# ImIntheMiddle/EmLoco

Hardware: AMD Instinct MI355X
Metric: env-steps/sec (SMPL humanoid, num_envs) (higher is better)
Workload: dtype f32

## Files before the change

### emloco_amd/csrc/emloco_types.h

```cpp
#pragma once
#define EMLOCO_PART_WORDS 416
#include "../../include/emloco_sim.h"
#define EMLOCO_PART_TAG(seq, part) ((seq) * 4u + (unsigned)(part))
#define EMLOCO_ERR_PART_TIMEOUT 1u

#define EMLOCO_TOPO_PARENT 0
#define EMLOCO_TOPO_DEPTH 24
#define EMLOCO_TOPO_CHILD 48
#define EMLOCO_TOPO_PDPACK 120
#define EMLOCO_TOPO_CAND 144
#define EMLOCO_TOPO_SCPAIR 240
#define EMLOCO_TOPO_WORDS 560

#define EMLOCO_MB_DYN 0
#define EMLOCO_MB_GEO 384
#define EMLOCO_MB_CAP 576
#define EMLOCO_MB_DRV 832
#define EMLOCO_MODEL_WORDS 1112

struct EmlocoSimDev {
    int n_env, n_cand, max_depth, sc_n;
    int sc_nseg;
    const int *topo;
    const float *model;
// ... 23 lines not shown
```

### emloco_amd/csrc/sim_capi.hip

```cpp
#include <hip/hip_runtime.h>
#include <cstdlib>
#include <cstdio>
#include <cstring>
#include <string>
#include <vector>
#ifdef EMLOCO_SIM_PAIR
#include "sim_pair_kernels.hip"
#define EMLOCO_SIM_ENVS_PER_WG 2
#else
#include "sim_kernels.hip"
#define EMLOCO_SIM_ENVS_PER_WG 1
#endif
#include "topology.h"
#include "model_pack.h"
#include "sim_state.h"

namespace {

thread_local std::string g_err;

int fail(int code, const char *what, hipError_t e = hipSuccess) {
    char buf[512];
    if (e != hipSuccess) snprintf(buf, sizeof(buf), "%s: %s", what, hipGetErrorString(e));
    else snprintf(buf, sizeof(buf), "%s", what);
// ... 343 lines not shown
    d.n_parts = dev_ids ? 1 : (s->n_parts < p.n_sub ? s->n_parts : p.n_sub);
    d.part_seq = ++s->part_seq; d.part_state = s->d_part_state.p; d.part_flag = s->d_part_flag.p;
    d.part_spin_max = s->part_spin_max; d.part_poison = s->part_poison;
    d.n_slots = dev_ids ? n_ids : s->n_env;
    const unsigned grid = (unsigned)(((d.n_slots + EMLOCO_SIM_ENVS_PER_WG - 1) / EMLOCO_SIM_ENVS_PER_WG) * d.n_parts);
    if (d.hf) hipLaunchKernelGGL(emloco::sim_step_kernel<1>, dim3(grid), dim3(64), (size_t)s->lds_pad, st, p, d);
    else hipLaunchKernelGGL(emloco::sim_step_kernel<0>, dim3(grid), dim3(64), (size_t)s->lds_pad, st, p, d);
    HIPCHK(hipGetLastError());
    if (timed) {
        HIPCHK(hipEventRecord(s->ev1[slot], st));
        s->ev_head = (slot + 1) % EmlocoSim::kRing;
        if (s->ev_count < EmlocoSim::kRing) ++s->ev_count;
    }
    return EMLOCO_OK;
}

int emloco_sim_set_split(EmlocoSim *s, int n_parts) {
    if (!s) return fail(EMLOCO_E_ARG, "emloco_sim_set_split: null sim");
    if (!s->prepared) return fail(EMLOCO_E_STATE, "emloco_sim_set_split: sim not prepared");
    if (n_parts < 1 || n_parts > 4) return fail(EMLOCO_E_ARG, "emloco_sim_set_split: 1 to 4 parts");
    if (n_parts > 1 && !s->d_part_state.p) {
        HIPCHK(hipSetDevice(s->device));
        HIPCHK(s->d_part_state.alloc((size_t)s->n_env * EMLOCO_PART_WORDS));
        HIPCHK(s->d_part_flag.alloc((size_t)s->n_env));
        HIPCHK(hipMemset(s->d_part_flag.p, 0, sizeof(unsigned) * (size_t)s->n_env));
    }
    s->n_parts = n_parts;
    return EMLOCO_OK;
}

int emloco_sim_set_cost_order(EmlocoSim *s, int on) {
    if (!s) return fail(EMLOCO_E_ARG, "emloco_sim_set_cost_order: null sim");
    if (!s->prepared) return fail(EMLOCO_E_STATE, "emloco_sim_set_cost_order: sim not prepared");
    if (on && !s->d_ticks.p) {
        HIPCHK(hipSetDevice(s->device));
        HIPCHK(s->d_ticks.alloc((size_t)s->n_env));
        HIPCHK(s->d_order.alloc((size_t)s->n_env));
        if (s->n_env > EMLOCO_ORDER_LDS_ENVS) HIPCHK(s->d_order_ws.alloc((size_t)s->n_env));
        HIPCHK(hipMemset(s->d_ticks.p, 0, sizeof(unsigned) * (size_t)s->n_env));
    }
    s->cost_order = on != 0;
    return EMLOCO_OK;
}

int emloco_sim_sync(EmlocoSim *s, void *stream) {
    if (!s) return fail(EMLOCO_E_ARG, "emloco_sim_sync: null sim");
// ... 26 lines not shown
int emloco_sim_set_root_state_indexed(EmlocoSim *s, const float *dev_full, const int32_t *ids, int n, void *stream) {
    return set_indexed(s, dev_full, s ? s->d_root.p : nullptr, 13, ids, n, stream);
}

int emloco_sim_set_dof_state_indexed(EmlocoSim *s, const float *dev_full, const int32_t *ids, int n, void *stream) {
    return set_indexed(s, dev_full, s ? s->d_dof.p : nullptr, EMLOCO_NDOF * 2, ids, n, stream);
}

int emloco_sim_refresh_bodies(EmlocoSim *s, void *stream) {
    if (!s) return fail(EMLOCO_E_ARG, "emloco_sim_refresh_bodies: null sim");
    if (!s->prepared) return fail(EMLOCO_E_STATE, "emloco_sim_refresh_bodies: sim not prepared");
    hipLaunchKernelGGL(emloco::sim_fk_kernel, dim3((unsigned)s->n_env), dim3(64), 0, (hipStream_t)stream, s->dev, (const int *)nullptr, s->n_env);
    HIPCHK(hipGetLastError());
    return EMLOCO_OK;
}

int emloco_sim_fk_indexed(EmlocoSim *s, const int32_t *ids, int n, void *stream) {
    if (!s || !s->prepared || !ids || n < 1) return fail(EMLOCO_E_ARG, "emloco_sim_fk_indexed: bad argument");
    hipLaunchKernelGGL(emloco::sim_fk_kernel, dim3((unsigned)(n > 256 ? 256 : n)), dim3(64), 0, (hipStream_t)stream, s->dev, (const int *)ids, n);
    HIPCHK(hipGetLastError());
    return EMLOCO_OK;
}

int emloco_sim_cost_ticks(EmlocoSim *s, unsigned *host_ticks, unsigned long long *host_start, int n) {
    if (!s || !host_ticks || n < 1 || !s->d_ticks.p) return fail(EMLOCO_E_ARG, "emloco_sim_cost_ticks: bad argument / cost order off");
    HIPCHK(hipDeviceSynchronize());
    const size_t m = (size_t)(n < s->n_env ? n : s->n_env);
    HIPCHK(hipMemcpy(host_ticks, s->d_ticks.p, sizeof(unsigned) * m, hipMemcpyDeviceToHost));
    if (host_start) {
        if (!s->dev.step_start) {
            unsigned long long *p = nullptr;
            HIPCHK(hipMalloc((void **)&p, sizeof(unsigned long long) * 2 * (size_t)s->n_env));
            HIPCHK(hipMemset(p, 0, sizeof(unsigned long long) * 2 * (size_t)s->n_env));
            s->dev.step_start = p;
        }
        HIPCHK(hipMemcpy(host_start, s->dev.step_start, sizeof(unsigned long long) * 2 * (size_t)s->n_env, hipMemcpyDeviceToHost));
    }
    return EMLOCO_OK;
}

int emloco_sim_profile(EmlocoSim *s, long long *host_out, int n) {
    if (!s || !host_out || n < 1) return fail(EMLOCO_E_ARG, "emloco_sim_profile: bad argument");
    if (!s->dev.prof) {
        long long *p = nullptr;
        HIPCHK(hipMalloc((void **)&p, 16 * 16 * sizeof(long long)));
        HIPCHK(hipMemset(p, 0, 16 * 16 * sizeof(long long)));
        s->dev.prof = p;
        return EMLOCO_OK;
    }
    HIPCHK(hipDeviceSynchronize());
    HIPCHK(hipMemcpy(host_out, s->dev.prof, sizeof(long long) * (n < 256 ? n : 256), hipMemcpyDeviceToHost));
    return EMLOCO_OK;
}

int emloco_sim_num_candidates(EmlocoSim *s) { return s ? s->topo.n_cand : EMLOCO_E_ARG; }

int emloco_sim_enable_timing(EmlocoSim *s, int on) {
    if (!s) return fail(EMLOCO_E_ARG, "emloco_sim_enable_timing: null sim");
    if (on && s->ev0.empty()) {
// ... 40 lines not shown
```

### emloco_amd/csrc/sim_kernels.hip

```cpp
#include <hip/hip_runtime.h>
#include "dev_math.h"
#include "sim_math.h"
#define cross3 fcross3
#define dot3 fdot3
#define dot6 fdot6
#define qmul fqmul
#define qnormalize fqnormalize
#define q2mat fq2mat
#define matvec3 fmatvec3
#define rotvec2quat frotvec2quat
#define quat2rotvec fquat2rotvec
#include "emloco_types.h"
#include "fk_device.h"
#include "order_device.h"

namespace emloco {

#define NB EMLOCO_NB
#define NDOF EMLOCO_NDOF
#define MAXC EMLOCO_MAXC
#define MAXR (3 * EMLOCO_MAXC)
#define MAXCAND EMLOCO_MAXCAND
#define EMLOCO_WH_MAX 1.0f
#define YLEN 30

__device__ __forceinline__ constexpr int sidx(int a, int b) {
    return a <= b ? (a * (13 - a)) / 2 + (b - a) : (b * (13 - b)) / 2 + (a - b);
}

__device__ __forceinline__ int tri_index(int a, int b) {
    const int hi = a > b ? a : b, lo = a > b ? b : a;
    return ((hi * (hi + 1)) >> 1) + lo;
}

struct ContactMatrixSquare { static constexpr bool square = true; };
struct ContactMatrixPacked { static constexpr bool square = false; };
template <bool SQ>
__device__ __forceinline__ void contact_entries3(const float *sh_A, int ao, int ls, int r, float &x0, float &x1, float &x2) {
    if (SQ) { x0 = sh_A[ao]; x1 = sh_A[ao + 1]; x2 = sh_A[ao + 2]; }
    else { x0 = sh_A[tri_index(ls, r)]; x1 = sh_A[tri_index(ls, r + 1)]; x2 = sh_A[tri_index(ls, r + 2)]; }
}

typedef float part_f4 __attribute__((ext_vector_type(4)));
#ifdef EMLOCO_EMU
__device__ __forceinline__ void part_st16(float *p, float a, float b, float c, float d) { p[0] = a; p[1] = b; p[2] = c; p[3] = d; }
__device__ __forceinline__ void part_ld16(const float *p, float *v) { for (int k = 0; k < 4; ++k) v[k] = p[k]; }
__device__ __forceinline__ void part_ld48(const float *p, float *v) { for (int g = 0; g < 3; ++g) for (int k = 0; k < 4; ++k) v[4 * g + k] = p[g * 4 * EMLOCO_NB + k]; }
__device__ __forceinline__ void part_stores_done() {}
__device__ __forceinline__ void part_flag_set(unsigned *f, unsigned v) { *f = v; }
__device__ __forceinline__ unsigned part_flag_get(const unsigned *f) { return *f; }
__device__ __forceinline__ void part_err_raise(unsigned *e, unsigned bit) { if (e) *e |= bit; }
#else
__device__ __forceinline__ void part_st16(float *p, float a, float b, float c, float d) {
    const part_f4 v = {a, b, c, d};
    asm volatile("global_store_dwordx4 %0, %1, off sc1" : : "v"(p), "v"(v) : "memory");
}
__device__ __forceinline__ void part_ld16(const float *p, float *v) {
    part_f4 a;
    asm volatile("global_load_dwordx4 %0, %1, off sc1\n\ts_waitcnt vmcnt(0)" : "=v"(a) : "v"(p) : "memory");
    v[0] = a.x; v[1] = a.y; v[2] = a.z; v[3] = a.w;
}
__device__ __forceinline__ void part_ld48(const float *p, float *v) {
    part_f4 a, b, c;
    static_assert(EMLOCO_NB * 16 == 384, "granule-major hand-over: a lane's three granules are 24 x 16 bytes apart");
    asm volatile("global_load_dwordx4 %0, %3, off sc1\n\tglobal_load_dwordx4 %1, %3, off offset:384 sc1\n\t"
                 "global_load_dwordx4 %2, %3, off offset:768 sc1\n\ts_waitcnt vmcnt(0)"
                 : "=&v"(a), "=&v"(b), "=&v"(c) : "v"(p) : "memory");
    v[0] = a.x; v[1] = a.y; v[2] = a.z; v[3] = a.w; v[4] = b.x; v[5] = b.y; v[6] = b.z; v[7] = b.w;
    v[8] = c.x; v[9] = c.y; v[10] = c.z; v[11] = c.w;
}
__device__ __forceinline__ void part_stores_done() { asm volatile("s_waitcnt vmcnt(0)" ::: "memory"); }
__device__ __forceinline__ void part_flag_set(unsigned *f, unsigned v) { __hip_atomic_store(f, v, __ATOMIC_RELAXED, __HIP_MEMORY_SCOPE_AGENT); }
__device__ __forceinline__ unsigned part_flag_get(const unsigned *f) { return __hip_atomic_load(f, __ATOMIC_RELAXED, __HIP_MEMORY_SCOPE_AGENT); }
__device__ __forceinline__ void part_err_raise(unsigned *e, unsigned bit) { if (e) __hip_atomic_fetch_or(e, bit, __ATOMIC_RELAXED, __HIP_MEMORY_SCOPE_SYSTEM); }
#endif

#ifdef EMLOCO_EMU
__device__ __forceinline__ void ld4(const float *base, int off, float *v) { for (int k = 0; k < 4; ++k) v[k] = base[off + k]; }
#else
__device__ __forceinline__ void ld4(const float *base, int off, float *v) {
    const part_f4 a = *(const part_f4 *)(base + off);
    v[0] = a.x; v[1] = a.y; v[2] = a.z; v[3] = a.w;
}
#endif

#ifdef EMLOCO_EMU
#define FRESH_LANE() do { } while (0)
#else
#define FRESH_LANE() asm volatile("" : "+v"(lane))
#endif
#define PD_PARENT(w) ((w) & 31)
#define PD_DEPTH(w) (((w) >> 5) & 15)
#define PD_SLOT(w) (((w) >> 9) & 7)
#define PD_CHILD(w, i) (((w) >> (12 + 5 * (i))) & 31)

#ifdef EMLOCO_SIM_PROFILE
#define PSTAMP(i) do { if (d.prof && env == 0 && lane == 0) d.prof[sub * 16 + (i)] = (long long)wall_clock64(); FRESH_LANE(); } while (0)
#else
#define PSTAMP(i) FRESH_LANE()
#endif

__device__ __forceinline__ void hf_plane(const EmlocoSimDev &d, float cx, float cy, float &zt, float n[3], int &id) {
    const float gx = (cx - d.hf_ox) * d.hf_inv_hs, gy = (cy - d.hf_oy) * d.hf_inv_hs;
    int i = (int)floorf(gx), j = (int)floorf(gy);
    i = i < 0 ? 0 : (i > d.hf_nx - 2 ? d.hf_nx - 2 : i);
    j = j < 0 ? 0 : (j > d.hf_ny - 2 ? d.hf_ny - 2 : j);
    const float u = gx - (float)i, v = gy - (float)j;
    id = ((i << 15) + j) * 2 + (u >= v ? 1 : 0);
    const short *c = d.hf + (long)i * d.hf_ny + j;
    const float h00 = d.hf_vs * (float)c[0], h01 = d.hf_vs * (float)c[1];
    const float h10 = d.hf_vs * (float)c[d.hf_ny], h11 = d.hf_vs * (float)c[d.hf_ny + 1];
    float zx, zy;
    if (u >= v) { zx = h10 - h00; zy = h11 - h10; } else { zy = h01 - h00; zx = h11 - h01; }
    zt = fmaf(v, zy, fmaf(u, zx, h00));
    const float sx = zx * d.hf_inv_hs, sy = zy * d.hf_inv_hs;
    const float inv = 1.0f / sqrtf(fmaf(sx, sx, fmaf(sy, sy, 1.0f)));
    n[0] = 0.0f - sx * inv; n[1] = 0.0f - sy * inv; n[2] = inv;
}
__device__ __forceinline__ int hf_triangle(const EmlocoSimDev &d, float cx, float cy) {
    const float gx = (cx - d.hf_ox) * d.hf_inv_hs, gy = (cy - d.hf_oy) * d.hf_inv_hs;
    int i = (int)floorf(gx), j = (int)floorf(gy);
    i = i < 0 ? 0 : (i > d.hf_nx - 2 ? d.hf_nx - 2 : i);
// ... 153 lines not shown
    signed char *sh_crange = (signed char *)(lds + O_CRANGE);
    unsigned char *sh_slot = (unsigned char *)(lds + O_SLOT);
    float (*sh_Ia)[24] = (float (*)[24])(lds + O_IA);
    float (*sh_cdir)[9] = (float (*)[9])(lds + O_IA);
    float (*sh_pa)[8] = (float (*)[8])(lds + O_PA);
    float (*sh_a)[8] = (float (*)[8])(lds + O_A_);
    float (*sh_V)[8] = (float (*)[8])(lds + O_V);
    float (*sh_Vf)[8] = (float (*)[8])(lds + O_VF);
    float (*sh_Aacc)[8] = (float (*)[8])(lds + O_AACC);
    float (*sh_fext)[8] = (float (*)[8])(lds + O_FEXT);
    float (*sh_pq)[8] = (float (*)[8])(lds + O_PQ);
    float *sh_A = lds + O_G;
    constexpr bool hf_on = HF != 0;

    const int *topo = d.topo;
    const float *mdl = d.model + (size_t)env * EMLOCO_MODEL_WORDS;
#define o_dyn (EMLOCO_MB_DYN + (lane < NB ? lane : 0) * 16)
#define jdof ((lane >= 1 && lane < NB) ? (lane - 1) * 3 : 0)
#define o_drv (EMLOCO_MB_DRV + jdof * 4)
    const float *tgt_env = d.pd_target + (size_t)env * NDOF;
    float *dofs_env = d.dof_state + (size_t)env * NDOF * 2;
    float *cf_env = d.contact_force + (size_t)env * NB * 3;
    float *lws_env = d.lambda_ws + (size_t)env * MAXCAND * 3;
    if (lane < NB) sh_pd[lane] = topo[EMLOCO_TOPO_PDPACK + lane];
    sh_slot[lane] = 255; sh_slot[lane + 64] = 255;

    const int sub_lo = (prm.n_sub * part) / n_parts, sub_hi = (prm.n_sub * (part + 1)) / n_parts;
    float *pst = d.part_state ? d.part_state + (long)env * EMLOCO_PART_WORDS : nullptr;
    float qj[4] = {0, 0, 0, 1}, wj[3] = {0, 0, 0}, edof[3] = {0, 0, 0};
    if (part == 0) {
        if ((lane < NB) && lane >= 1) {
            const float *ds = dofs_env + jdof * 2;
            float e[3] = {ds[0], ds[2], ds[4]};
            rotvec2quat(e, qj);
            wj[0] = ds[1]; wj[1] = ds[3]; wj[2] = ds[5];
            quat2rotvec(qj, edof);
        }
        if (lane == 0) {
            const float *rs = d.root_state + (long)env * 13;
            float q0[4] = {rs[3], rs[4], rs[5], rs[6]};
            qnormalize(q0);
            for (int k = 0; k < 3; ++k) { sh_root[k] = rs[k]; sh_root[7 + k] = rs[10 + k]; sh_root[10 + k] = rs[7 + k]; }
            for (int k = 0; k < 4; ++k) sh_root[3 + k] = q0[k];
        }
    } else {
        if (lane == 0) {
            int spins = 0;
            const unsigned want = EMLOCO_PART_TAG(d.part_seq, part - 1);
            while (part_flag_get(d.part_flag + env) != want && ++spins < d.part_spin_max) __builtin_amdgcn_s_sleep(16);
            sh_V0[0] = spins < d.part_spin_max ? 1.0f : 0.0f;
            if (spins >= d.part_spin_max) part_err_raise(d.err, EMLOCO_ERR_PART_TIMEOUT);
        }
        __syncthreads();
        if (sh_V0[0] == 0.0f) { work = -1; return; }
        __syncthreads();
        if ((lane < NB)) {
            float v[12];
            part_ld48(pst + lane * 4, v);
            for (int k = 0; k < 4; ++k) qj[k] = v[k];
            for (int k = 0; k < 3; ++k) wj[k] = v[4 + k];
            edof[0] = v[7]; edof[1] = v[8]; edof[2] = v[9];
        } else if (lane < NB + 32) {
            const int g = lane - NB;
            float v[4];
            part_ld16(pst + NB * 12 + 4 * g, v);
            float *dst = g < 4 ? sh_root + 4 * g : g < 6 ? sh_P + 4 * (g - 4) : g < 22 ? sh_lam + 4 * (g - 6) : g < 30 ? (float *)sh_slot + 4 * (g - 22) : sh_L;
            if (g != 30) for (int k = 0; k < 4; ++k) dst[k] = v[k];
            else sh_V0[0] = v[0];
        }
        __syncthreads();
        work = __float_as_int(sh_V0[0]);
    }
    __syncthreads();

    const float h = prm.h;
    float tau[3], dd[3];
    int sat[3];
    float uh[3], qdd[3];

    for (int sub = sub_lo; sub < sub_hi + (part == n_parts - 1 ? 1 : 0); ++sub) {
        const bool final_pass = (sub == prm.n_sub);
        const bool last = (sub == prm.n_sub - 1);

        PSTAMP(0);
        if (lane == 0) {
            float q0[4] = {sh_root[3], sh_root[4], sh_root[5], sh_root[6]}, R[9];
            q2mat(q0, R);
            for (int k = 0; k < 3; ++k) { sh_pq[0][k] = sh_root[k]; sh_R[0][9 + k] = 0.0f; }
            for (int k = 0; k < 4; ++k) sh_pq[0][4 + k] = q0[k];
            for (int k = 0; k < 9; ++k) sh_R[0][k] = R[k];
            for (int k = 0; k < 6; ++k) { sh_V[0][k] = sh_root[7 + k]; sh_Aacc[0][k] = 0.0f; }
        }
        float jm[4];
        ld4(mdl, o_dyn, jm);
        const float joff[3] = {jm[0], jm[1], jm[2]};
        __syncthreads();
        const int pd1 = sh_pd[lane < NB ? lane : 0];
        for (int lev = 1; lev <= d.max_depth; ++lev) {
            if ((lane < NB) && PD_DEPTH(pd1) == lev) {
                const int p = PD_PARENT(pd1);
                float Rp[9], o[3], qp[4], qw[4], pw[3], R[9], r[3], Sl[3][3], V[6];
                for (int k = 0; k < 9; ++k) Rp[k] = sh_R[p][k];
                for (int k = 0; k < 4; ++k) qp[k] = sh_pq[p][4 + k];
                matvec3(Rp, joff, o);
                for (int k = 0; k < 3; ++k) { pw[k] = sh_pq[p][k] + o[k]; r[k] = pw[k] - sh_root[k]; }
                qmul(qp, qj, qw);
                qnormalize(qw);
                q2mat(qw, R);
                float wv[3], Vp[6];
                for (int k = 0; k < 6; ++k) Vp[k] = sh_V[p][k];
                for (int c = 0; c < 3; ++c) {
                    float ax[3] = {R[c], R[3 + c], R[6 + c]};
                    cross3(r, ax, Sl[c]);
                }
                for (int k = 0; k < 3; ++k) {
                    wv[k] = SOP3(R[k * 3], wj[0], R[k * 3 + 1], wj[1], R[k * 3 + 2], wj[2]);
                    V[k] = Vp[k] + wv[k];
// ... 128 lines not shown
                    const float b0 = sh_L[0] - Lact[0], b1 = sh_L[1] - Lact[1], b2 = sh_L[2] - Lact[2];
                    const float c00 = Jc[1] * Jc[2] - Jc[5] * Jc[5], c01 = Jc[4] * Jc[5] - Jc[3] * Jc[2], c02 = Jc[3] * Jc[5] - Jc[4] * Jc[1];
                    const float c11 = Jc[0] * Jc[2] - Jc[4] * Jc[4], c12 = Jc[3] * Jc[4] - Jc[0] * Jc[5], c22 = Jc[0] * Jc[1] - Jc[3] * Jc[3];
                    const float det = SOP3(Jc[0], c00, Jc[3], c01, Jc[4], c02);
                    if (det > 1e-12f) {
                        dw[0] = SOP3(c00, b0, c01, b1, c02, b2) / det;
                        dw[1] = SOP3(c01, b0, c11, b1, c12, b2) / det;
                        dw[2] = SOP3(c02, b0, c12, b1, c22, b2) / det;
                        cross3(Cc, dw, dvO);
                        moved = true;
                    }
                }
                __syncthreads();
                if (moved && (lane < NB))
                    for (int k = 0; k < 3; ++k) { sh_V[lane][k] = Vn[k] + dw[k]; sh_V[lane][3 + k] = Vn[3 + k] + dvO[k]; }
                if (lane == 0) {
                    if (moved) for (int k = 0; k < 3; ++k) { sh_root[7 + k] += dw[k]; sh_root[10 + k] += dvO[k]; }
                    for (int k = 0; k < 3; ++k) { sh_L[4 + k] = moved ? sh_L[k] : Lact[k]; sh_L[8 + k] = Cc[k]; }
                }
                __syncthreads();
            }
        }
        if (final_pass) break;

        if (d.sc_n > 0) {
            float *sh_seg = sh_A;
            float *sh_hitw = sh_A + EMLOCO_SC_MAXSEG * 8;
            int *sh_hitb = (int *)(sh_A + EMLOCO_SC_MAXSEG * 8 + EMLOCO_SC_MAXHITS * 6);
            if (lane < d.sc_nseg) {
                float R[9], r[3], ca[4], cb[4], pa[3], pb[3];
                ld4(mdl, EMLOCO_MB_CAP + lane * 8, ca); ld4(mdl, EMLOCO_MB_CAP + lane * 8 + 4, cb);
                const int sb = (int)cb[3];
                for (int k = 0; k < 9; ++k) R[k] = sh_R[sb][k];
                for (int k = 0; k < 3; ++k) r[k] = sh_R[sb][9 + k];
                matvec3(R, ca, pa); matvec3(R, cb, pb);
                for (int k = 0; k < 3; ++k) { sh_seg[lane * 8 + k] = r[k] + pa[k]; sh_seg[lane * 8 + 3 + k] = r[k] + pb[k]; }
                sh_seg[lane * 8 + 6] = ca[3];
                const float ax[3] = {pb[0] - pa[0], pb[1] - pa[1], pb[2] - pa[2]};
                sh_seg[lane * 8 + 7] = 0.5f * sqrtf(ax[0] * ax[0] + ax[1] * ax[1] + ax[2] * ax[2]);
            }
            __syncthreads();
            int *sh_cand = (int *)(sh_A + EMLOCO_SC_MAXSEG * 8 + EMLOCO_SC_MAXHITS * 8);
            int ncand = 0;
            for (int q0 = 0; q0 < d.sc_n; q0 += 64) {
                const int q = q0 + lane;
                bool keep = false;
// ... 65 lines not shown
                if (hit && slot < EMLOCO_SC_MAXHITS) {
                    for (int k = 0; k < 6; ++k) sh_hitw[slot * 6 + k] = w6[k];
                    sh_hitb[slot * 2] = bi; sh_hitb[slot * 2 + 1] = bj;
                }
                nh += __popcll(bal);
            }
            if (nh > EMLOCO_SC_MAXHITS) nh = EMLOCO_SC_MAXHITS;
            __syncthreads();
            if ((lane < NB)) {
                float fe[6] = {0, 0, 0, 0, 0, 0};
                for (int hh = 0; hh < nh; ++hh) {
                    const int bi = sh_hitb[hh * 2], bj = sh_hitb[hh * 2 + 1];
                    if (bi == lane) for (int k = 0; k < 6; ++k) fe[k] += sh_hitw[hh * 6 + k];
                    else if (bj == lane) for (int k = 0; k < 6; ++k) fe[k] -= sh_hitw[hh * 6 + k];
                }
                for (int k = 0; k < 6; ++k) sh_fext[lane][k] = fe[k];
            }
            __syncthreads();
        }

        PSTAMP(1);
        if ((lane < NB)) {
            for (int k = 0; k < 3; ++k) {
                float dr[4];
                ld4(mdl, o_drv + 4 * k, dr);
                const float kp = lane >= 1 ? dr[0] : 0.0f, kd = lane >= 1 ? dr[1] : 0.0f;
                const float arm = lane >= 1 ? dr[2] : 0.0f, tgt = lane >= 1 ? tgt_env[jdof + k] : 0.0f;
                const float e = tgt - edof[k];
                if (prm.drive_mode == 1) {
                    const float eff = lane >= 1 ? dr[3] : 0.0f;
                    sat[k] = 2; tau[k] = tgt > eff ? eff : (tgt < -eff ? -eff : tgt); dd[k] = arm;
                } else {
                    sat[k] = 0; tau[k] = kp * e - (kd + h * kp) * wj[k]; dd[k] = arm + h * kd + h * h * kp;
                }
            }
        }

        PSTAMP(2);
#if defined(EMLOCO_DUMMY_VALU) || defined(EMLOCO_DUMMY_LDS) || defined(EMLOCO_DUMMY_SALU)
        {
#ifdef EMLOCO_DUMMY_VALU
            float z0 = h, z1 = h + 1.0f, z2 = h + 2.0f, z3 = h + 3.0f;
            for (int i = 0; i < EMLOCO_DUMMY_VALU / 4; ++i)
                asm volatile("v_fma_f32 %0, %0, %0, %1\n\tv_fma_f32 %1, %1, %1, %2\n\tv_fma_f32 %2, %2, %2, %3\n\tv_fma_f32 %3, %3, %3, %0"
                             : "+v"(z0), "+v"(z1), "+v"(z2), "+v"(z3));
            if (z0 + z1 + z2 + z3 == 12345.678f) sh_V0[11] = z0;
#endif
#ifdef EMLOCO_DUMMY_LDS
            part_f4 q0, q1, q2, q3;
            const unsigned la = (unsigned)(lane & 15) * 48u + (unsigned)(O_R * 4);
            for (int i = 0; i < EMLOCO_DUMMY_LDS / 4; ++i)
                asm volatile("ds_read_b128 %0, %4\n\tds_read_b128 %1, %4 offset:16\n\tds_read_b128 %2, %4 offset:32\n\tds_read_b128 %3, %4 offset:64\n\ts_waitcnt lgkmcnt(0)"
                             : "=v"(q0), "=v"(q1), "=v"(q2), "=v"(q3) : "v"(la) : "memory");
            if (q0.x + q1.x + q2.x + q3.x == 12345.678f) sh_V0[11] = q0.x;
#endif
#ifdef EMLOCO_DUMMY_SALU
            int c0 = sub, c1 = sub + 1;
            for (int i = 0; i < EMLOCO_DUMMY_SALU / 4; ++i)
                asm volatile("s_add_i32 %0, %0, %1\n\ts_xor_b32 %1, %1, %0\n\ts_add_i32 %0, %0, 7\n\ts_xor_b32 %1, %1, 5" : "+s"(c0), "+s"(c1));
            if (c0 + c1 == 123456789) sh_V0[11] = 1.0f;
#endif
        }
#endif
        float pA[6];
        for (int pass = 0; pass < 2; ++pass) {
        float IA[21];
        for (int k = 0; k < 21; ++k) IA[k] = 0.0f;
        if ((lane < NB)) {
            float R[9], r[3], V[6];
            for (int k = 0; k < 9; ++k) R[k] = sh_R[lane][k];
            for (int k = 0; k < 3; ++k) r[k] = sh_R[lane][9 + k];
            for (int k = 0; k < 6; ++k) V[k] = sh_V[lane][k];
            float Rc[9], Ic[9], cw[3], c[3], in6[8], bcom[4];
            ld4(mdl, o_dyn + 8, in6); ld4(mdl, o_dyn + 12, in6 + 4);
            ld4(mdl, o_dyn + 4, bcom);
            const float bmass = mdl[o_dyn + 3];
            const float Ib[9] = {in6[0], in6[3], in6[4], in6[3], in6[1], in6[5], in6[4], in6[5], in6[2]};
            for (int a = 0; a < 3; ++a)
                for (int q = 0; q < 3; ++q) Rc[a * 3 + q] = SOP3(R[a * 3], Ib[q], R[a * 3 + 1], Ib[3 + q], R[a * 3 + 2], Ib[6 + q]);
            for (int a = 0; a < 3; ++a)
                for (int q = a; q < 3; ++q) {
                    Ic[a * 3 + q] = SOP3(Rc[a * 3], R[q * 3], Rc[a * 3 + 1], R[q * 3 + 1], Rc[a * 3 + 2], R[q * 3 + 2]);
                    Ic[q * 3 + a] = Ic[a * 3 + q];
                }
            matvec3(R, bcom, cw);
            for (int k = 0; k < 3; ++k) c[k] = r[k] + cw[k];
            const float ms = bmass, cc = dot3(c, c);
// ... 87 lines not shown
                        }
                    float y[6], x[6];
                    for (int a = 0; a < 6; ++a) {
                        float acc = -pA[a];
                        for (int k = 0; k < a; ++k) acc = fmaf(-LT(a, k), y[k], acc);
                        y[a] = acc * Li[a];
                    }
                    for (int a = 5; a >= 0; --a) {
                        float acc = y[a];
                        for (int k = a + 1; k < 6; ++k) acc = fmaf(-LT(k, a), x[k], acc);
                        x[a] = acc * Li[a];
                    }
                    for (int a = 0; a < 6; ++a)
                        for (int q = 0; q <= a; ++q) sh_L0[a * 6 + q] = LT(a, q);
                    for (int a = 0; a < 6; ++a) sh_L0i[a] = Li[a];
#undef LT
                    for (int k = 0; k < 6; ++k) sh_a[0][k] = x[k];
                }
            }
            __syncthreads();
        }

        PSTAMP(3);
        const int pd4 = sh_pd[lane < NB ? lane : 0];
        for (int lev = 1; lev <= d.max_depth; ++lev) {
            if ((lane < NB) && PD_DEPTH(pd4) == lev) {
                float ap[6], t[3], a[6], Wm[18], Km[6];
                float R[9], r[3], Sl[3][3];
                for (int k = 0; k < 9; ++k) R[k] = sh_R[lane][k];
                for (int k = 0; k < 3; ++k) r[k] = sh_R[lane][9 + k];
                for (int c = 0; c < 3; ++c) { const float ax[3] = {R[c], R[3 + c], R[6 + c]}; cross3(r, ax, Sl[c]); }
                for (int k = 0; k < 18; ++k) Wm[k] = sh_W[lane][k];
                for (int k = 0; k < 6; ++k) Km[k] = sh_W[lane][18 + k];
                for (int k = 0; k < 6; ++k) ap[k] = sh_a[PD_PARENT(pd4)][k];
                for (int c = 0; c < 3; ++c) {
                    float acc = 0.0f;
                    for (int k = 0; k < 6; ++k) acc = fmaf(Wm[k * 3 + c], ap[k], acc);
                    t[c] = uh[c] - acc;
                }
                qdd[0] = SOP3(Km[0], t[0], Km[1], t[1], Km[3], t[2]);
                qdd[1] = SOP2(Km[2], t[1], Km[4], t[2]);
                qdd[2] = Km[5] * t[2];
                for (int k = 0; k < 3; ++k) {
                    a[k] = ADD_SOP3(ap[k], R[k * 3], qdd[0], R[k * 3 + 1], qdd[1], R[k * 3 + 2], qdd[2]);
                    a[3 + k] = ADD_SOP3(ap[3 + k], Sl[0][k], qdd[0], Sl[1][k], qdd[1], Sl[2][k], qdd[2]);
                }
                for (int k = 0; k < 6; ++k) sh_a[lane][k] = a[k];
            }
            __syncthreads();
        }
        if (pass == 0) {
            bool over = false;
            if ((lane < NB) && lane >= 1)
                for (int k = 0; k < 3; ++k) {
                    float dr[4];
                    ld4(mdl, o_drv + 4 * k, dr);
                    const float kp = dr[0], kd = dr[1], eff = dr[3];
                    const float ti = tau[k] - (h * kd + h * h * kp) * qdd[k];
                    if (sat[k] == 0 && fabsf(ti) > eff) { sat[k] = ti > 0.0f ? 1 : -1; tau[k] = ti > 0.0f ? eff : -eff; dd[k] = dr[2]; over = true; }
                }
            if (__ballot(over) == 0ull) break;
        }
        }
        if ((lane < NB)) {
            for (int k = 0; k < 6; ++k) sh_Vf[lane][k] = fmaf(h, sh_a[lane][k], sh_V[lane][k]);
            if (lane == 0) for (int k = 0; k < 6; ++k) { sh_V0[k] = fmaf(h, sh_a[0][k], sh_root[7 + k]); sh_V0[6 + k] = 0.0f; }
        }

        PSTAMP(4);
        float *sh_stage = lds + O_G;
        static_assert(O_VF - O_G >= 128 * 7, "candidate staging does not fit the arrays that are dead in phase 5");
        int cb[2]; float cdist[2]; bool act[2];
        for (int s = 0; s < 2; ++s) {
            const int c = lane + 64 * s;
            cb[s] = -1; act[s] = false; cdist[s] = 0.0f;
            if (c < d.n_cand) {
                const int cp = topo[EMLOCO_TOPO_CAND + c], body = cp & 0xff, k = (cp >> 8) & 0xff, gt = cp >> 16;
                float ga[4], gb[4], clp[3];
                ld4(mdl, EMLOCO_MB_GEO + body * 8, ga); ld4(mdl, EMLOCO_MB_GEO + body * 8 + 4, gb);
                const float crad = ga[3];
                cb[s] = body;
                if (gt == EMLOCO_GEOM_SPHERE) { clp[0] = ga[0]; clp[1] = ga[1]; clp[2] = ga[2]; }
                else if (gt == EMLOCO_GEOM_CAPSULE) {
                    const float *src = k == 0 ? ga : gb;
                    clp[0] = src[0]; clp[1] = src[1]; clp[2] = src[2];
                } else {
                    clp[0] = ga[0] + ((k & 1) ? gb[0] : -gb[0]);
                    clp[1] = ga[1] + ((k & 2) ? gb[1] : -gb[1]);
                    clp[2] = ga[2] + ((k & 4) ? gb[2] : -gb[2]);
                }
                float Rb[9], wp[3], cxw[3];
                for (int k2 = 0; k2 < 9; ++k2) Rb[k2] = sh_R[body][k2];
                matvec3(Rb, clp, wp);
                const float z = sh_pq[body][2] + wp[2];
                float *stg = sh_stage + c * 7;
                if (!hf_on) {
                    cdist[s] = (z - prm.ground_z) - crad;
                    cxw[0] = sh_R[body][9] + wp[0];
                    cxw[1] = sh_R[body][10] + wp[1];
                    cxw[2] = (sh_R[body][11] + wp[2]) - crad;
// ... 472 lines not shown
        }
        if (lane == 0) {
            float V0[6];
            for (int k = 0; k < 6; ++k) V0[k] = sh_V0[k] + sh_V0[6 + k];
            for (int k = 0; k < 3; ++k) V0[k] *= damp;
            const float n = sqrtf(dot3(V0, V0));
            if (n > prm.max_ang_vel) { const float sc = prm.max_ang_vel / n; V0[0] *= sc; V0[1] *= sc; V0[2] *= sc; clamped = true; }
            float e[3], dqt[4], qn[4], q0[4] = {sh_root[3], sh_root[4], sh_root[5], sh_root[6]};
            for (int k = 0; k < 3; ++k) { sh_root[k] += h * V0[3 + k]; e[k] = h * V0[k]; }
            rotvec2quat(e, dqt);
            qmul(dqt, q0, qn); qnormalize(qn);
            for (int k = 0; k < 4; ++k) sh_root[3 + k] = qn[k];
            float wxv[3];
            cross3(V0, V0 + 3, wxv);
            for (int k = 0; k < 3; ++k) V0[3 + k] = fmaf(h, wxv[k], V0[3 + k]);
            for (int k = 0; k < 6; ++k) sh_root[7 + k] = V0[k];
        }
        {
            const bool any_clamped = __ballot(clamped) != 0ull;
            if (lane == 0) sh_L[3] = any_clamped ? 0.0f : 1.0f;
        }
        __syncthreads();
        PSTAMP(10);
    }

    if (part < n_parts - 1) {
        if ((lane < NB)) {
            float *ps = pst + lane * 4;
            part_st16(ps, qj[0], qj[1], qj[2], qj[3]);
            part_st16(ps + 4 * NB, wj[0], wj[1], wj[2], edof[0]);
            part_st16(ps + 8 * NB, edof[1], edof[2], 0.0f, 0.0f);
        } else if (lane < NB + 32) {
            const int g = lane - NB;
            const float *src = g < 4 ? sh_root + 4 * g : g < 6 ? sh_P + 4 * (g - 4) : g < 22 ? sh_lam + 4 * (g - 6) : g < 30 ? (const float *)sh_slot + 4 * (g - 22) : sh_L;
            if (g != 30) part_st16(pst + NB * 12 + 4 * g, src[0], src[1], src[2], src[3]);
            else part_st16(pst + NB * 12 + 4 * g, __int_as_float(work), 0.0f, 0.0f, 0.0f);
        }
        part_stores_done();
        __syncthreads();
        if (lane == 0 && !(part == 0 && env == d.part_poison)) part_flag_set(d.part_flag + env, EMLOCO_PART_TAG(d.part_seq, part));
        return;
    }
    if ((lane < NB)) {
        float *o = d.rb_state + (size_t)env * NB * 13 + lane * 13;
        float t[3], V[6], r[3];
        for (int k = 0; k < 6; ++k) V[k] = sh_V[lane][k];
        for (int k = 0; k < 3; ++k) r[k] = sh_R[lane][9 + k];
        cross3(V, r, t);
        for (int k = 0; k < 3; ++k) { o[k] = sh_pq[lane][k]; o[7 + k] = V[3 + k] + t[k]; o[10 + k] = V[k]; }
        for (int k = 0; k < 4; ++k) o[3 + k] = sh_pq[lane][4 + k];
        if (lane >= 1) {
            float *ds = dofs_env + jdof * 2;
            for (int k = 0; k < 3; ++k) { ds[2 * k] = edof[k]; ds[2 * k + 1] = wj[k]; }
        }
    }
    if (lane == 0) {
        float *rs = d.root_state + (long)env * 13;
        for (int k = 0; k < 3; ++k) { rs[k] = sh_root[k]; rs[7 + k] = sh_root[10 + k]; rs[10 + k] = sh_root[7 + k]; }
        for (int k = 0; k < 4; ++k) rs[3 + k] = sh_root[3 + k];
    }
    for (int s = 0; s < 2; ++s) {
        const int c = lane + 64 * s;
        if (c < MAXCAND) {
// ... 5 lines not shown
#undef o_dyn
#undef jdof
#undef o_drv

template <int HF>
__global__ void __attribute__((amdgpu_flat_work_group_size(64, 64), amdgpu_waves_per_eu(EMLOCO_SIM_WAVES_PER_SIMD, EMLOCO_SIM_WAVES_PER_SIMD)))
sim_step_kernel(EmlocoSimParams prm, EmlocoSimDev d) {
    const int n_parts = d.n_parts > 1 ? d.n_parts : 1;
    const int part = (int)blockIdx.x / d.n_env, slot = (int)blockIdx.x - part * d.n_env;
    if (part >= n_parts) return;
    int env = d.step_order ? d.step_order[slot] : slot;
    if (d.step_ids) { env = d.step_ids[slot]; if (env < 0) return; }
    if (d.step_skip && d.step_skip[env] != 0) return;
    env = __builtin_amdgcn_readfirstlane(env);
    const long long t0 = d.step_start ? (long long)wall_clock64() : 0ll;
    int work;
    sim_step_env<HF>(prm, d, env, work, part, n_parts);
    if (d.step_ticks && threadIdx.x == 0 && part == n_parts - 1) {
#ifdef EMLOCO_COST_KEY_TICKS
        d.step_ticks[env] = (unsigned)(((long long)wall_clock64() - t0) >> 9);
#else
        d.step_ticks[env] = (unsigned)work;
#endif
        if (d.step_start) { d.step_start[env] = (unsigned long long)t0; d.step_start[d.n_env + env] = (unsigned long long)wall_clock64(); }
    }
}

__global__ void __launch_bounds__(1024)
sim_order_kernel(const unsigned *ticks, int n, int *order, unsigned char *bucket_ws) {
    order_sort(ticks, n, order, bucket_ws);
}

__global__ void __launch_bounds__(64)
sim_fk_kernel(EmlocoSimDev d, const int *env_ids, int n_ids) {
    const int lane = threadIdx.x;
    for (int bi = blockIdx.x; bi < n_ids; bi += gridDim.x) {
        const int env = env_ids ? env_ids[bi] : bi;
        if (env < 0) break;
        __shared__ float sm[FK_SM_FLOATS];
        fk_env(d, env, lane, sm);
        __syncthreads();
    }
}

__global__ void __launch_bounds__(64)
copy_rows_kernel(const float *src, float *dst, const int *ids, int n_ids, int row_len, int n_env) {
    const int i = blockIdx.x;
    if (i >= n_ids) return;
// ... 18 lines not shown
```

Baseline: 9.670 million.

## Replace flag-based part hand-over with tagged self-validating state words

The multi-part hand-over no longer writes the state, waits for the stores and then sets a separate flag that lane 0 spins on. Each value is now interleaved with the sequence tag, so the consumer lanes poll the state block directly and check it with a wave ballot. This removes a store drain, a flag round-trip and several barriers, at the cost of a doubled hand-over buffer and wider loads per poll. Model loads (joint offsets, drive params, candidate words, PD words) are also hoisted out of inner loops, and an optional scheduling timestamp probe is added.

```diff
diff --git a/emloco_amd/csrc/emloco_types.h b/emloco_amd/csrc/emloco_types.h
--- a/emloco_amd/csrc/emloco_types.h
+++ b/emloco_amd/csrc/emloco_types.h
@@ -1,5 +1,5 @@
 #pragma once
-#define EMLOCO_PART_WORDS 416
+#define EMLOCO_PART_WORDS 800
 #include "../../include/emloco_sim.h"
 #define EMLOCO_PART_TAG(seq, part) ((seq) * 4u + (unsigned)(part))
 #define EMLOCO_ERR_PART_TIMEOUT 1u
diff --git a/emloco_amd/csrc/sim_capi.hip b/emloco_amd/csrc/sim_capi.hip
--- a/emloco_amd/csrc/sim_capi.hip
+++ b/emloco_amd/csrc/sim_capi.hip
@@ -389,6 +389,7 @@
     if (n_parts > 1 && !s->d_part_state.p) {
         HIPCHK(hipSetDevice(s->device));
         HIPCHK(s->d_part_state.alloc((size_t)s->n_env * EMLOCO_PART_WORDS));
+        HIPCHK(hipMemset(s->d_part_state.p, 0, sizeof(float) * (size_t)s->n_env * EMLOCO_PART_WORDS));
         HIPCHK(s->d_part_flag.alloc((size_t)s->n_env));
         HIPCHK(hipMemset(s->d_part_flag.p, 0, sizeof(unsigned) * (size_t)s->n_env));
     }
@@ -461,6 +462,11 @@
     return EMLOCO_OK;
 }
 
+#ifdef EMLOCO_SIM_SCHED
+#define EMLOCO_STEP_START_WORDS 16
+#else
+#define EMLOCO_STEP_START_WORDS 2
+#endif
 int emloco_sim_cost_ticks(EmlocoSim *s, unsigned *host_ticks, unsigned long long *host_start, int n) {
     if (!s || !host_ticks || n < 1 || !s->d_ticks.p) return fail(EMLOCO_E_ARG, "emloco_sim_cost_ticks: bad argument / cost order off");
     HIPCHK(hipDeviceSynchronize());
@@ -469,11 +475,11 @@
     if (host_start) {
         if (!s->dev.step_start) {
             unsigned long long *p = nullptr;
-            HIPCHK(hipMalloc((void **)&p, sizeof(unsigned long long) * 2 * (size_t)s->n_env));
-            HIPCHK(hipMemset(p, 0, sizeof(unsigned long long) * 2 * (size_t)s->n_env));
+            HIPCHK(hipMalloc((void **)&p, sizeof(unsigned long long) * EMLOCO_STEP_START_WORDS * (size_t)s->n_env));
+            HIPCHK(hipMemset(p, 0, sizeof(unsigned long long) * EMLOCO_STEP_START_WORDS * (size_t)s->n_env));
             s->dev.step_start = p;
         }
-        HIPCHK(hipMemcpy(host_start, s->dev.step_start, sizeof(unsigned long long) * 2 * (size_t)s->n_env, hipMemcpyDeviceToHost));
+        HIPCHK(hipMemcpy(host_start, s->dev.step_start, sizeof(unsigned long long) * EMLOCO_STEP_START_WORDS * (size_t)s->n_env, hipMemcpyDeviceToHost));
     }
     return EMLOCO_OK;
 }
diff --git a/emloco_amd/csrc/sim_kernels.hip b/emloco_amd/csrc/sim_kernels.hip
--- a/emloco_amd/csrc/sim_kernels.hip
+++ b/emloco_amd/csrc/sim_kernels.hip
@@ -42,36 +42,32 @@
 }
 
 typedef float part_f4 __attribute__((ext_vector_type(4)));
+#define PART_G1 (64 * 4)
+#define PART_GB (128 * 4)
+static_assert(EMLOCO_PART_WORDS >= PART_GB + 3 * EMLOCO_NB * 4, "hand-over block too small for its layout");
 #ifdef EMLOCO_EMU
 __device__ __forceinline__ void part_st16(float *p, float a, float b, float c, float d) { p[0] = a; p[1] = b; p[2] = c; p[3] = d; }
-__device__ __forceinline__ void part_ld16(const float *p, float *v) { for (int k = 0; k < 4; ++k) v[k] = p[k]; }
-__device__ __forceinline__ void part_ld48(const float *p, float *v) { for (int g = 0; g < 3; ++g) for (int k = 0; k < 4; ++k) v[4 * g + k] = p[g * 4 * EMLOCO_NB + k]; }
-__device__ __forceinline__ void part_stores_done() {}
-__device__ __forceinline__ void part_flag_set(unsigned *f, unsigned v) { *f = v; }
-__device__ __forceinline__ unsigned part_flag_get(const unsigned *f) { return *f; }
+__device__ __forceinline__ void part_ld80(const float *pa, const float *pb, float *v) {
+    for (int k = 0; k < 4; ++k) { v[k] = pa[k]; v[4 + k] = pa[PART_G1 + k]; }
+    for (int g = 0; g < 3; ++g) for (int k = 0; k < 4; ++k) v[8 + 4 * g + k] = pb[g * 4 * EMLOCO_NB + k];
+}
 __device__ __forceinline__ void part_err_raise(unsigned *e, unsigned bit) { if (e) *e |= bit; }
 #else
 __device__ __forceinline__ void part_st16(float *p, float a, float b, float c, float d) {
     const part_f4 v = {a, b, c, d};
     asm volatile("global_store_dwordx4 %0, %1, off sc1" : : "v"(p), "v"(v) : "memory");
 }
-__device__ __forceinline__ void part_ld16(const float *p, float *v) {
-    part_f4 a;
-    asm volatile("global_load_dwordx4 %0, %1, off sc1\n\ts_waitcnt vmcnt(0)" : "=v"(a) : "v"(p) : "memory");
-    v[0] = a.x; v[1] = a.y; v[2] = a.z; v[3] = a.w;
-}
-__device__ __forceinline__ void part_ld48(const float *p, float *v) {
-    part_f4 a, b, c;
-    static_assert(EMLOCO_NB * 16 == 384, "granule-major hand-over: a lane's three granules are 24 x 16 bytes apart");
-    asm volatile("global_load_dwordx4 %0, %3, off sc1\n\tglobal_load_dwordx4 %1, %3, off offset:384 sc1\n\t"
-                 "global_load_dwordx4 %2, %3, off offset:768 sc1\n\ts_waitcnt vmcnt(0)"
-                 : "=&v"(a), "=&v"(b), "=&v"(c) : "v"(p) : "memory");
+__device__ __forceinline__ void part_ld80(const float *pa, const float *pb, float *v) {
+    part_f4 a, b, c, e, f;
+    static_assert(PART_G1 * 4 == 1024 && EMLOCO_NB * 16 == 384, "granule-major hand-over: the offsets of a lane's granules");
+    asm volatile("global_load_dwordx4 %0, %5, off sc1\n\tglobal_load_dwordx4 %1, %5, off offset:1024 sc1\n\t"
+                 "global_load_dwordx4 %2, %6, off sc1\n\tglobal_load_dwordx4 %3, %6, off offset:384 sc1\n\t"
+                 "global_load_dwordx4 %4, %6, off offset:768 sc1\n\ts_waitcnt vmcnt(0)"
+                 : "=&v"(a), "=&v"(b), "=&v"(c), "=&v"(e), "=&v"(f) : "v"(pa), "v"(pb) : "memory");
     v[0] = a.x; v[1] = a.y; v[2] = a.z; v[3] = a.w; v[4] = b.x; v[5] = b.y; v[6] = b.z; v[7] = b.w;
-    v[8] = c.x; v[9] = c.y; v[10] = c.z; v[11] = c.w;
-}
-__device__ __forceinline__ void part_stores_done() { asm volatile("s_waitcnt vmcnt(0)" ::: "memory"); }
-__device__ __forceinline__ void part_flag_set(unsigned *f, unsigned v) { __hip_atomic_store(f, v, __ATOMIC_RELAXED, __HIP_MEMORY_SCOPE_AGENT); }
-__device__ __forceinline__ unsigned part_flag_get(const unsigned *f) { return __hip_atomic_load(f, __ATOMIC_RELAXED, __HIP_MEMORY_SCOPE_AGENT); }
+    v[8] = c.x; v[9] = c.y; v[10] = c.z; v[11] = c.w; v[12] = e.x; v[13] = e.y; v[14] = e.z; v[15] = e.w;
+    v[16] = f.x; v[17] = f.y; v[18] = f.z; v[19] = f.w;
+}
 __device__ __forceinline__ void part_err_raise(unsigned *e, unsigned bit) { if (e) __hip_atomic_fetch_or(e, bit, __ATOMIC_RELAXED, __HIP_MEMORY_SCOPE_SYSTEM); }
 #endif
 
@@ -98,6 +94,12 @@
 #define PSTAMP(i) do { if (d.prof && env == 0 && lane == 0) d.prof[sub * 16 + (i)] = (long long)wall_clock64(); FRESH_LANE(); } while (0)
 #else
 #define PSTAMP(i) FRESH_LANE()
+#endif
+
+#ifdef EMLOCO_SIM_SCHED
+#define SCHED_HANDED() do { if (d.step_start && threadIdx.x == 0) d.step_start[((size_t)part * d.n_env + env) * 4 + 1] = (unsigned long long)wall_clock64(); } while (0)
+#else
+#define SCHED_HANDED() do { } while (0)
 #endif
 
 __device__ __forceinline__ void hf_plane(const EmlocoSimDev &d, float cx, float cy, float &zt, float n[3], int &id) {
@@ -297,7 +299,9 @@
     float *dofs_env = d.dof_state + (size_t)env * NDOF * 2;
     float *cf_env = d.contact_force + (size_t)env * NB * 3;
     float *lws_env = d.lambda_ws + (size_t)env * MAXCAND * 3;
-    if (lane < NB) sh_pd[lane] = topo[EMLOCO_TOPO_PDPACK + lane];
+    const int pd_w = lane < NB ? topo[EMLOCO_TOPO_PDPACK + lane] : 0;
+    float jm[4];
+    ld4(mdl, o_dyn, jm);
     sh_slot[lane] = 255; sh_slot[lane + 64] = 255;
 
     const int sub_lo = (prm.n_sub * part) / n_parts, sub_hi = (prm.n_sub * (part + 1)) / n_parts;
@@ -319,34 +323,39 @@
             for (int k = 0; k < 4; ++k) sh_root[3 + k] = q0[k];
         }
     } else {
-        if (lane == 0) {
-            int spins = 0;
-            const unsigned want = EMLOCO_PART_TAG(d.part_seq, part - 1);
-            while (part_flag_get(d.part_flag + env) != want && ++spins < d.part_spin_max) __builtin_amdgcn_s_sleep(16);
-            sh_V0[0] = spins < d.part_spin_max ? 1.0f : 0.0f;
-            if (spins >= d.part_spin_max) part_err_raise(d.err, EMLOCO_ERR_PART_TIMEOUT);
-        }
-        __syncthreads();
-        if (sh_V0[0] == 0.0f) { work = -1; return; }
-        __syncthreads();
+        const unsigned want = EMLOCO_PART_TAG(d.part_seq, part - 1);
+        const float *pa = pst + lane * 4, *pb = lane < NB ? pst + PART_GB + lane * 4 : pa;
+        float v[20];
+        int spins = 0;
+        bool bad;
+        for (;;) {
+            part_ld80(pa, pb, v);
+            bool miss = __float_as_uint(v[1]) != want || __float_as_uint(v[3]) != want || __float_as_uint(v[5]) != want || __float_as_uint(v[7]) != want;
+            if (lane < NB)
+                for (int k = 9; k < 20; k += 2) miss = miss || __float_as_uint(v[k]) != want;
+            bad = __ballot(miss) != 0ull;
+            if (!bad || ++spins >= d.part_spin_max) break;
+            __builtin_amdgcn_s_sleep(16);
+        }
+        if (bad) {
+            if (lane == 0) part_err_raise(d.err, EMLOCO_ERR_PART_TIMEOUT);
+            work = -1;
+            return;
+        }
         if ((lane < NB)) {
-            float v[12];
-            part_ld48(pst + lane * 4, v);
-            for (int k = 0; k < 4; ++k) qj[k] = v[k];
-            for (int k = 0; k < 3; ++k) wj[k] = v[4 + k];
-            edof[0] = v[7]; edof[1] = v[8]; edof[2] = v[9];
+            qj[0] = v[0]; qj[1] = v[2]; qj[2] = v[4]; qj[3] = v[6];
+            wj[0] = v[8]; wj[1] = v[10]; wj[2] = v[12];
+            edof[0] = v[14]; edof[1] = v[16]; edof[2] = v[18];
         } else if (lane < NB + 32) {
             const int g = lane - NB;
-            float v[4];
-            part_ld16(pst + NB * 12 + 4 * g, v);
             float *dst = g < 4 ? sh_root + 4 * g : g < 6 ? sh_P + 4 * (g - 4) : g < 22 ? sh_lam + 4 * (g - 6) : g < 30 ? (float *)sh_slot + 4 * (g - 22) : sh_L;
-            if (g != 30) for (int k = 0; k < 4; ++k) dst[k] = v[k];
-            else sh_V0[0] = v[0];
-        }
-        __syncthreads();
-        work = __float_as_int(sh_V0[0]);
+            if (g != 30) { dst[0] = v[0]; dst[1] = v[2]; dst[2] = v[4]; dst[3] = v[6]; }
+        }
+        work = __shfl(__float_as_int(v[0]), NB + 30);
     }
+    if (lane < NB) sh_pd[lane] = pd_w;
     __syncthreads();
+    SCHED_HANDED();
 
     const float h = prm.h;
     float tau[3], dd[3];
@@ -366,8 +375,6 @@
             for (int k = 0; k < 9; ++k) sh_R[0][k] = R[k];
             for (int k = 0; k < 6; ++k) { sh_V[0][k] = sh_root[7 + k]; sh_Aacc[0][k] = 0.0f; }
         }
-        float jm[4];
-        ld4(mdl, o_dyn, jm);
         const float joff[3] = {jm[0], jm[1], jm[2]};
         __syncthreads();
         const int pd1 = sh_pd[lane < NB ? lane : 0];
@@ -542,6 +549,9 @@
             }
         }
         if (final_pass) break;
+        float drv[3][4] = {{0, 0, 0, 0}, {0, 0, 0, 0}, {0, 0, 0, 0}}, tgv[3] = {0, 0, 0};
+        if ((lane < NB))
+            for (int k = 0; k < 3; ++k) { ld4(mdl, o_drv + 4 * k, drv[k]); tgv[k] = tgt_env[jdof + k]; }
 
         if (d.sc_n > 0) {
             float *sh_seg = sh_A;
@@ -653,10 +663,9 @@
         PSTAMP(1);
         if ((lane < NB)) {
             for (int k = 0; k < 3; ++k) {
-                float dr[4];
-                ld4(mdl, o_drv + 4 * k, dr);
+                const float *dr = drv[k];
                 const float kp = lane >= 1 ? dr[0] : 0.0f, kd = lane >= 1 ? dr[1] : 0.0f;
-                const float arm = lane >= 1 ? dr[2] : 0.0f, tgt = lane >= 1 ? tgt_env[jdof + k] : 0.0f;
+                const float arm = lane >= 1 ? dr[2] : 0.0f, tgt = lane >= 1 ? tgv[k] : 0.0f;
                 const float e = tgt - edof[k];
                 if (prm.drive_mode == 1) {
                     const float eff = lane >= 1 ? dr[3] : 0.0f;
@@ -694,6 +703,7 @@
         }
 #endif
         float pA[6];
+        int cand_w[2] = {0, 0};
         for (int pass = 0; pass < 2; ++pass) {
         float IA[21];
         for (int k = 0; k < 21; ++k) IA[k] = 0.0f;
@@ -827,6 +837,10 @@
         }
 
         PSTAMP(3);
+        float drc[3][4] = {{0, 0, 0, 0}, {0, 0, 0, 0}, {0, 0, 0, 0}};
+        if (pass == 0 && (lane < NB) && lane >= 1)
+            for (int k = 0; k < 3; ++k) ld4(mdl, o_drv + 4 * k, drc[k]);
+        for (int s = 0; s < 2; ++s) cand_w[s] = lane + 64 * s < d.n_cand ? topo[EMLOCO_TOPO_CAND + lane + 64 * s] : 0;
         const int pd4 = sh_pd[lane < NB ? lane : 0];
         for (int lev = 1; lev <= d.max_depth; ++lev) {
             if ((lane < NB) && PD_DEPTH(pd4) == lev) {
@@ -858,8 +872,7 @@
             bool over = false;
             if ((lane < NB) && lane >= 1)
                 for (int k = 0; k < 3; ++k) {
-                    float dr[4];
-                    ld4(mdl, o_drv + 4 * k, dr);
+                    const float *dr = drc[k];
                     const float kp = dr[0], kd = dr[1], eff = dr[3];
                     const float ti = tau[k] - (h * kd + h * h * kp) * qdd[k];
                     if (sat[k] == 0 && fabsf(ti) > eff) { sat[k] = ti > 0.0f ? 1 : -1; tau[k] = ti > 0.0f ? eff : -eff; dd[k] = dr[2]; over = true; }
@@ -880,7 +893,7 @@
             const int c = lane + 64 * s;
             cb[s] = -1; act[s] = false; cdist[s] = 0.0f;
             if (c < d.n_cand) {
-                const int cp = topo[EMLOCO_TOPO_CAND + c], body = cp & 0xff, k = (cp >> 8) & 0xff, gt = cp >> 16;
+                const int cp = cand_w[s], body = cp & 0xff, k = (cp >> 8) & 0xff, gt = cp >> 16;
                 float ga[4], gb[4], clp[3];
                 ld4(mdl, EMLOCO_MB_GEO + body * 8, ga); ld4(mdl, EMLOCO_MB_GEO + body * 8 + 4, gb);
                 const float crad = ga[3];
@@ -1399,23 +1412,29 @@
         }
         __syncthreads();
         PSTAMP(10);
+        ld4(mdl, o_dyn, jm);
     }
 
     if (part < n_parts - 1) {
-        if ((lane < NB)) {
-            float *ps = pst + lane * 4;
-            part_st16(ps, qj[0], qj[1], qj[2], qj[3]);
-            part_st16(ps + 4 * NB, wj[0], wj[1], wj[2], edof[0]);
-            part_st16(ps + 8 * NB, edof[1], edof[2], 0.0f, 0.0f);
-        } else if (lane < NB + 32) {
+        if (part == 0 && env == d.part_poison) return;
+        const float tg = __uint_as_float(EMLOCO_PART_TAG(d.part_seq, part));
+        float w[4] = {0.0f, 0.0f, 0.0f, 0.0f};
+        if ((lane < NB)) { w[0] = qj[0]; w[1] = qj[1]; w[2] = qj[2]; w[3] = qj[3]; }
+        else if (lane < NB + 32) {
             const int g = lane - NB;
             const float *src = g < 4 ? sh_root + 4 * g : g < 6 ? sh_P + 4 * (g - 4) : g < 22 ? sh_lam + 4 * (g - 6) : g < 30 ? (const float *)sh_slot + 4 * (g - 22) : sh_L;
-            if (g != 30) part_st16(pst + NB * 12 + 4 * g, src[0], src[1], src[2], src[3]);
-            else part_st16(pst + NB * 12 + 4 * g, __int_as_float(work), 0.0f, 0.0f, 0.0f);
-        }
-        part_stores_done();
-        __syncthreads();
-        if (lane == 0 && !(part == 0 && env == d.part_poison)) part_flag_set(d.part_flag + env, EMLOCO_PART_TAG(d.part_seq, part));
+            if (g != 30) { w[0] = src[0]; w[1] = src[1]; w[2] = src[2]; w[3] = src[3]; }
+            else w[0] = __int_as_float(work);
+        }
+        float *pa = pst + lane * 4;
+        part_st16(pa, w[0], tg, w[1], tg);
+        part_st16(pa + PART_G1, w[2], tg, w[3], tg);
+        if ((lane < NB)) {
+            float *pb = pst + PART_GB + lane * 4;
+            part_st16(pb, wj[0], tg, wj[1], tg);
+            part_st16(pb + 4 * NB, wj[2], tg, edof[0], tg);
+            part_st16(pb + 8 * NB, edof[1], tg, edof[2], tg);
+        }
         return;
     }
     if ((lane < NB)) {
@@ -1467,8 +1486,16 @@
 #else
         d.step_ticks[env] = (unsigned)work;
 #endif
+#ifndef EMLOCO_SIM_SCHED
         if (d.step_start) { d.step_start[env] = (unsigned long long)t0; d.step_start[d.n_env + env] = (unsigned long long)wall_clock64(); }
+#endif
     }
+#ifdef EMLOCO_SIM_SCHED
+    if (d.step_start && threadIdx.x == 0) {
+        unsigned long long *ss = d.step_start + ((size_t)part * d.n_env + env) * 4;
+        ss[0] = (unsigned long long)t0; ss[2] = (unsigned long long)wall_clock64(); ss[3] = (unsigned long long)(part | slot << 8);
+    }
+#endif
 }
 
 __global__ void __launch_bounds__(1024)
```

Result: faster. 9.800 million (median of 6 runs) (+1.3%).
